# Mictronics/multi-sdr-gps-sim

Hardware: NVIDIA H100
Metric: IQ Msamples/s (higher is better)
Workload: dtype f64 NCO / int32 accumulate / int8 out

## Files before the change

multi-sdr-gps-sim_b200/csrc/synth_lanes.cu:

```cuda
#include <cuda_runtime.h>
#include <stdint.h>

#include "nco_exact.h"
#include "synth_kernels.h"
#include "synth_lanes.h"

namespace gpsb200 {

namespace {

constexpr int kLaneWarps = 16;
constexpr int kLaneChipWords = 36;

struct LaneWin {
    uint32_t s0, s1, s2;
    uint32_t base;
};

struct LaneSteps {
    uint64_t D96, E96;
    uint32_t inv32, e22;
};

template <int CH>
struct LanesSmem {
    static constexpr int kWins = 32 / CH;
    uint32_t chips[CH][kLaneChipWords];
    uint32_t nav[CH][kNavWords];
    alignas(16) LaneWin win[kLaneWarps][kWins][CH];
    alignas(16) uint32_t step[CH];
    LaneSteps steps[CH];
    alignas(16) uint32_t stage[kLaneWarps][kWins * lanes::kWindow];
    uint32_t band[CH][lanes::kBandList + 1];
};
template <int CH>
constexpr size_t lanes_smem_bytes() { return sizeof(LanesSmem<CH>) + (size_t) CH * 2048 + 2048; }

template <int OFF>
__device__ __forceinline__ int table_at(uint32_t p, uint32_t ta) {
    int e;
    asm volatile("{\n\t.reg .b32 i, ad;\n\tshr.b32 i, %1, 23;\n\tmad.lo.u32 ad, i, 4, %2;\n\tld.shared.b32 %0, [ad+%3];\n\t}"
                 : "=r"(e)
                 : "r"(p), "r"(ta), "n"(OFF));
    return e;
}

template <class ChipFn, class NavFn>
__device__ __noinline__ uint3 exact_signs_call(lanes::Anchor an, int w, ChipFn chips, NavFn nav) {
    uint32_t W[3];
    lanes::exact_signs(an, w, chips, nav, W);
    return make_uint3(W[0], W[1], W[2]);
}

__device__ __noinline__ int exact_index_call(lanes::Anchor an, int w, int n) {
    const uint64_t D = lanes::carr_step_fix(an.c);
    const uint64_t P = lanes::carr_fix(an.x0) + (uint64_t) w * ((uint64_t) lanes::kWindow * D);
    return lanes::exact_index(P, D, an, w, n);
}

__device__ __forceinline__ void add_if(int &acc, uint32_t w, uint32_t bit, int e) {
    asm("{\n\t.reg .pred p;\n\t.reg .b32 t;\n\tand.b32 t, %1, %2;\n\tsetp.ne.u32 p, t, 0;\n\t@p add.s32 %0, %0, %3;\n\t}"
        : "+r"(acc)
        : "r"(w), "r"(bit), "r"(e));
}

template <bool IQ16, int CH>
__global__ void __launch_bounds__(kLaneWarps * 32, 2) k_synth_lanes(SynthArgs a) {
    constexpr int WINS = 32 / CH;
    constexpr int SWZ = 32 / CH;
    extern __shared__ __align__(16) unsigned char smem_raw[];
    const uint32_t raw_base = (uint32_t) __cvta_generic_to_shared(smem_raw);
    const uint32_t tab_base = (raw_base + 2047u) & ~2047u;
    int32_t *tab = reinterpret_cast<int32_t *>(smem_raw + (tab_base - raw_base));
    LanesSmem<CH> &sm = *reinterpret_cast<LanesSmem<CH> *>(smem_raw + (tab_base - raw_base) + CH * 2048);
    constexpr uint32_t kFull = 0xFFFFFFFFu;

    const int b = blockIdx.x / a.ctas_per_block;
    const int g = blockIdx.x - b * a.ctas_per_block;
    const int tid = threadIdx.x, nthr = blockDim.x;
    const int lane = tid & 31, warp = tid >> 5;
    const int nchan = a.nchan;
    const BlockChanDev *bc = a.bc + (size_t) b * nchan;

    {
        const int32_t *src = a.atab + (size_t) b * kAtabRows * 32;
        for (int i = tid; i < 512 * CH; i += nthr) {
            const int k = i / CH, c = i - k * CH;
            tab[c * 512 + ((k + c * SWZ) & 511)] = c < nchan ? src[k * 32 + c] : 0;
        }
        for (int i = tid; i < CH * kLaneChipWords; i += nthr) {
            const int c = i / kLaneChipWords, w = i - c * kLaneChipWords;
            uint32_t v = 0;
            if (c < nchan && bc[c].prn > 0) {
                const uint32_t *cw = a.chipbits + bc[c].prn * kChipWords;
                v = w < kChipWords ? cw[w] : __funnelshift_r(cw[w - 32], cw[w - 31], 1);
            }
            sm.chips[c][w] = v;
        }
        for (int i = tid; i < CH * kNavWords; i += nthr) {
            const int c = i / kNavWords, w = i - c * kNavWords;
            uint32_t v = 0;
            if (c < nchan && bc[c].prn > 0) v = a.nav[((size_t) bc[c].frame * a.nav_stride + c) * kNavWords + w];
            sm.nav[c][w] = v;
        }
        if (warp == kLaneWarps - 1 && lane < CH) {
            const bool ok = lane < nchan && bc[lane].prn > 0;
            lanes::ChanRun k;
            lanes::init_steps(k, ok, ok ? bc[lane].c_carr : 0.0, ok ? bc[lane].c_code : 0.0);
            sm.steps[lane] = LaneSteps{k.D96, k.E96, k.inv32, k.e22};
            sm.step[lane] = lanes::fast_step(k);
            lanes::band_residues(lanes::fast_step(k), &sm.band[lane][0]);
        }
    }
    __syncthreads();

    const int ch = lane & (CH - 1), half = lane / CH;
    const bool chan_ok = ch < nchan && bc[ch < nchan ? ch : 0].prn > 0;
    const uint32_t *nav_row = &sm.nav[ch][0];
    const uint32_t *chip_row = &sm.chips[ch][0];
    const uint32_t *band_row = &sm.band[ch][0];
    auto navf = [nav_row](int iw) { return nav_row[iw]; };
    auto chipf = [chip_row](int i) { return chip_row[i]; };
    const uint32_t n0 = (uint32_t) lane, n1 = n0 + 32u, n2 = n0 + 64u;
    const uint32_t sbit = 1u << lanes::sign_pos(lane);
    const int nwin = a.run_samples / lanes::kWindow;
    uint32_t *stage = &sm.stage[warp][0];

    const int run_first = g * a.runs_per_cta;
    const int run_last = min(run_first + a.runs_per_cta, a.nruns);
#pragma unroll 1
    for (int r = run_first + warp; r < run_last; r += kLaneWarps) {
        auto anchor = [&](int c) {
            const RunCkpt k0 = a.ck[((size_t) b * a.nruns + r) * nchan + c];
            return lanes::Anchor{k0.x, k0.y, bc[c].c_carr, bc[c].c_code, k0.nav};
        };
        lanes::ChanRun s;
        auto load_steps = [&]() {
            const LaneSteps k = sm.steps[ch];
            s.D96 = k.D96;
            s.E96 = k.E96;
            s.inv32 = k.inv32;
            s.e22 = k.e22;
        };
        {
            const lanes::Anchor an = chan_ok ? anchor(ch) : lanes::Anchor{0.0, 0.0, 0.0, 0.0, 0u};
            lanes::init_run(s, chan_ok, an.x0, an.y0, an.navpos, an.c, an.d, navf);
        }
        if (WINS == 2 && chan_ok && half == 1) {
            load_steps();
            lanes::advance_window(s, navf);
        }
        const size_t samp0 = (size_t) b * kBlockSamples + (size_t) r * a.run_samples;

#pragma unroll 1
        for (int w = 0; w < nwin; w += WINS) {
            uint32_t flagged;
            {
                uint32_t S[3] = {0u, 0u, 0u};
                uint32_t base = (uint32_t) (ch * SWZ) << 23;
                bool band = false;
                if (chan_ok) load_steps();
                if (chan_ok && w > 0) {
#pragma unroll
                    for (int i = 0; i < WINS; i++) lanes::advance_window(s, navf);
                }
                if (chan_ok && w + half < nwin) {
                    base += lanes::fast_base(s);
                    band = lanes::window_band_risky(band_row, base);
                    if (!lanes::window_signs(s, chipf, navf, S)) {
                        const uint3 e = exact_signs_call(anchor(ch), w + half, chipf, navf);
                        S[0] = e.x;
                        S[1] = e.y;
                        S[2] = e.z;
                    }
                }
                *reinterpret_cast<uint4 *>(&sm.win[warp][half][ch]) = make_uint4(S[0], S[1], S[2], base);
                flagged = __ballot_sync(kFull, band);
            }
            __syncwarp();

#pragma unroll
            for (int hh = 0; hh < WINS; hh++) {
                if (w + hh >= nwin) break;
                const LaneWin *wrow = &sm.win[warp][hh][0];
                int all0 = 0, all1 = 0, all2 = 0, neg0 = 0, neg1 = 0, neg2 = 0;
                const LaneWin *wp = wrow;
                const uint32_t *sp = &sm.step[0];
                uint32_t ta = tab_base;
#pragma unroll 4
                for (int c = 0; c < nchan; c += 2, wp += 2, sp += 2, ta += 2 * 2048u) {
                    const uint4 wa = *reinterpret_cast<const uint4 *>(&wp[0]);
                    const uint4 wb = *reinterpret_cast<const uint4 *>(&wp[1]);
                    const uint2 st = *reinterpret_cast<const uint2 *>(sp);
                    const uint32_t a0 = wa.w + n0 * st.x, a1 = wa.w + n1 * st.x, a2 = wa.w + n2 * st.x;
                    const uint32_t b0 = wb.w + n0 * st.y, b1 = wb.w + n1 * st.y, b2 = wb.w + n2 * st.y;
                    const int ea0 = table_at<0>(a0, ta), eb0 = table_at<2048>(b0, ta);
                    const int ea1 = table_at<0>(a1, ta), eb1 = table_at<2048>(b1, ta);
                    const int ea2 = table_at<0>(a2, ta), eb2 = table_at<2048>(b2, ta);
                    all0 += ea0 + eb0;
                    all1 += ea1 + eb1;
                    all2 += ea2 + eb2;
                    add_if(neg0, wa.x, sbit, ea0);
                    add_if(neg0, wb.x, sbit, eb0);
                    add_if(neg1, wa.y, sbit, ea1);
                    add_if(neg1, wb.y, sbit, eb1);
                    add_if(neg2, wa.z, sbit, ea2);
                    add_if(neg2, wb.z, sbit, eb2);
                }
                int accs[3] = {(int) ((uint32_t) all0 - 2u * (uint32_t) neg0), (int) ((uint32_t) all1 - 2u * (uint32_t) neg1),
                               (int) ((uint32_t) all2 - 2u * (uint32_t) neg2)};
                for (uint32_t m = WINS == 1 ? flagged : (flagged >> (hh * CH)) & 0xFFFFu; m != 0u; m &= m - 1u) {
                    const int c = __ffs((int) m) - 1;
                    const uint4 wv = *reinterpret_cast<const uint4 *>(&wrow[c]);
                    const uint32_t st = sm.step[c];
                    const uint32_t p0 = wv.w + n0 * st, p1 = wv.w + n1 * st, p2 = wv.w + n2 * st;
                    const bool risky = lanes::fast_risky(p0) | lanes::fast_risky(p1) | lanes::fast_risky(p2);
                    if (!risky) continue;
                    const lanes::Anchor ac = anchor(c);
                    const uint32_t ps[3] = {p0, p1, p2}, sw[3] = {wv.x, wv.y, wv.z};
#pragma unroll
                    for (int j = 0; j < 3; j++) {
                        if (!lanes::fast_risky(ps[j])) continue;
                        const int kf = (int) (ps[j] >> 23);
                        const int k = exact_index_call(ac, w + hh, 32 * j + lane);
                        const int fix = tab[c * 512 + ((k + c * SWZ) & 511)] - tab[c * 512 + kf];
                        accs[j] += (sw[j] & sbit) ? -fix : fix;
                    }
                }
#pragma unroll
                for (int j = 0; j < 3; j++) {
                    const int p = accs[j];
                    const int iv = (int) (short) (p & 0xFFFF);
                    const int qv = (p - iv) >> 16;
                    const int n = hh * lanes::kWindow + 32 * j + lane;
                    if (IQ16) {
                        stage[n] = ((uint32_t) iv & 0xFFFFu) | ((uint32_t) qv << 16);
                    } else {
                        reinterpret_cast<uint16_t *>(stage)[n] =
                            (uint16_t) ((((uint32_t) (iv >> 4)) & 0xFFu) | ((((uint32_t) (qv >> 4)) & 0xFFu) << 8));
                    }
                }
            }
            __syncwarp();
            {
                const int nsamp = (nwin - w >= WINS ? WINS : 1) * lanes::kWindow;
                const int nvec = nsamp * (IQ16 ? 4 : 2) / 16;
                uint4 *dst = reinterpret_cast<uint4 *>(reinterpret_cast<char *>(a.out) +
                                                       (samp0 + (size_t) w * lanes::kWindow) * (IQ16 ? 4 : 2));
                const uint4 *srcv = reinterpret_cast<const uint4 *>(stage);
                for (int i = lane; i < nvec; i += 32) dst[i] = srcv[i];
            }
        }
    }
}

}

bool synth_lanes_applicable(const SynthArgs &a) {
    return a.lanes && a.nchan <= 32 && a.run_samples % lanes::kWindow == 0 && a.run_samples <= lanes::kMaxRun;
}

static int device_sms() {
    int dev = 0, n = 0;
    if (cudaGetDevice(&dev) != cudaSuccess || cudaDeviceGetAttribute(&n, cudaDevAttrMultiProcessorCount, dev) != cudaSuccess)
        return 132;
    return n;
}

static void lanes_shape(const SynthArgs &a, int *ctas_per_block, int *runs_per_cta) {
    int per_block = (40 * 2 * device_sms() + a.nblk - 1) / a.nblk;
    if (per_block > 16) per_block = 16;
    if (per_block < 1) per_block = 1;
    int per_cta = (a.nruns + per_block - 1) / per_block;
    per_cta = (per_cta + kLaneWarps - 1) / kLaneWarps * kLaneWarps;
    per_block = (a.nruns + per_cta - 1) / per_cta;
    *ctas_per_block = per_block;
    *runs_per_cta = per_cta;
}

template <bool IQ16, int CH>
static cudaError_t launch_lanes_t(const SynthArgs &a, cudaStream_t s) {
    const size_t smem = lanes_smem_bytes<CH>();
    cudaError_t e = cudaFuncSetAttribute(k_synth_lanes<IQ16, CH>, cudaFuncAttributeMaxDynamicSharedMemorySize, (int) smem);
    if (e != cudaSuccess) return e;
    k_synth_lanes<IQ16, CH><<<a.nblk * a.ctas_per_block, kLaneWarps * 32, smem, s>>>(a);
    return cudaGetLastError();
}

cudaError_t launch_synth_lanes(const SynthArgs &a_in, cudaStream_t s) {
    SynthArgs a = a_in;
    lanes_shape(a, &a.ctas_per_block, &a.runs_per_cta);
    if (a.nchan <= 16) return a.iq16 ? launch_lanes_t<true, 16>(a, s) : launch_lanes_t<false, 16>(a, s);
    return a.iq16 ? launch_lanes_t<true, 32>(a, s) : launch_lanes_t<false, 32>(a, s);
}

void synth_lanes_launch_shape(const SynthArgs &a, int *ctas, int *threads, size_t *smem, int *ctas_per_block,
                              int *runs_per_cta) {
    int per_block, per_cta;
    lanes_shape(a, &per_block, &per_cta);
    *ctas = a.nblk * per_block;
    *threads = kLaneWarps * 32;
    *smem = a.nchan <= 16 ? lanes_smem_bytes<16>() : lanes_smem_bytes<32>();
    *ctas_per_block = per_block;
    *runs_per_cta = per_cta;
}

}
```

multi-sdr-gps-sim_b200/csrc/synth_lanes.h:

```cpp
#pragma once
#include <stdint.h>

#include "nco_exact.h"

namespace gpsb200 {
namespace lanes {

constexpr int kWindow = 96;
constexpr int kMaxRun = 2400;
constexpr uint64_t kOne54 = 1ull << 54;
constexpr uint64_t kCodeWrap54 = 1023ull << 54;
constexpr uint64_t kBandCode = 1ull << 22;
constexpr uint64_t kBandCarr = 1ull << 23;
constexpr uint32_t kBandFast = 128;

GPSB_HD bool code_step_ok(double c_code) { return c_code >= 0.33855 && c_code < 0.34340; }

GPSB_HD uint64_t carr_fix(double x) { return (x >= 0.0 && x < 1.0) ? (uint64_t) (x * 0x1p64) : 0; }
GPSB_HD uint64_t carr_step_fix(double c) {
    const double a = c < 0.0 ? -c : c;
    const uint64_t m = (uint64_t) (a * 0x1p64);
    return c < 0.0 ? (uint64_t) 0 - m : m;
}
GPSB_HD uint64_t code_fix(double y) { return (uint64_t) (y * 0x1p54); }

GPSB_HD uint32_t funnel_r(uint32_t lo, uint32_t hi, int sh) {
#if defined(__CUDA_ARCH__)
    return __funnelshift_r(lo, hi, sh);
#else
    return sh ? (lo >> sh) | (hi << (32 - sh)) : lo;
#endif
}

struct ChanRun {
    uint64_t P, D;
    uint64_t Y, E;
    uint64_t D96, E96;
    uint32_t inv32;
    uint32_t e22;
    int iword, ibit, icode, dbit;
    bool active;
};

struct Anchor {
    double x0, y0, c, d;
    uint32_t navpos;
};

template <class NavFn>
GPSB_HD int nav_bit_at(NavFn nav, int iw, int ib) {
    const uint32_t w = nav(iw < 60 ? iw : 59);
    return (int) ((w >> (29 - ib)) & 1u);
}

GPSB_HD void init_steps(ChanRun &s, bool active, double c, double d) {
    s.D = carr_step_fix(c);
    s.E = code_fix(d);
    s.D96 = (uint64_t) kWindow * s.D;
    s.E96 = (uint64_t) kWindow * s.E;
    const uint64_t d3 = 3 * s.E - kOne54;
    s.inv32 = active ? (uint32_t) (0x1p79 / (double) d3) : 0u;
    s.e22 = (uint32_t) (s.E >> 22);
}

template <class NavFn>
GPSB_HD void init_run(ChanRun &s, bool active, double x, double y, uint32_t navpos, double c, double d, NavFn nav) {
    s.active = active;
    s.iword = (int) (navpos & 0xFF);
    s.ibit = (int) ((navpos >> 8) & 0xFF);
    s.icode = (int) ((navpos >> 16) & 0xFF);
    s.P = carr_fix(x);
    s.Y = code_fix(y);
    init_steps(s, active, c, d);
    s.dbit = active ? nav_bit_at(nav, s.iword, s.ibit) : 0;
}

GPSB_HD uint32_t mulhi32(uint32_t a, uint32_t b) {
#if defined(__CUDA_ARCH__)
    return __umulhi(a, b);
#else
    return (uint32_t) (((uint64_t) a * b) >> 32);
#endif
}

GPSB_HD bool window_signs_fp64(const ChanRun &s, uint32_t c_lo, uint32_t c_hi, int j0, uint32_t S[3]) {
    const uint64_t d3 = (s.E96 >> 5) - kOne54;
    const double rinv = 1.0 / (double) d3;
    const double tband = (double) kBandCode * rinv + 0x1p-40;
    bool certain = true;
#pragma unroll
    for (int r = 0; r < 3; r++) {
        const uint64_t phi = s.Y + (uint64_t) r * s.E;
        const int J = (int) (phi >> 54) - j0;
        const uint64_t F = phi & (kOne54 - 1);
        const double t = (double) (kOne54 - F) * rinv;
        const double tf = t < 64.0 ? (double) (int) t : 64.0;
        const int qs = (int) tf + 1;
        certain &= F >= kBandCode;
        if (qs <= 32) certain &= (t - tf >= tband) & (tf + 1.0 - t >= tband);
        const uint32_t lowm = qs >= 32 ? 0xFFFFFFFFu : ((1u << qs) - 1u);
        const uint32_t a = funnel_r(c_lo, c_hi, J), b = funnel_r(c_lo, c_hi, J + 1);
        S[r] = (a & lowm) | (b & ~lowm);
    }
    return certain;
}

GPSB_HD int sign_pos(int i) { return 11 * (i % 3) + i / 3; }

GPSB_HD void sample_words(const uint32_t S[3], uint32_t W[3]) {
    W[0] = (S[0] & 0x7FFu) | ((S[1] & 0x7FFu) << 11) | (S[2] << 22);
    W[1] = ((S[2] >> 10) & 0x7FFu) | (((S[0] >> 11) & 0x7FFu) << 11) | ((S[1] >> 11) << 22);
    W[2] = (S[1] >> 21) | ((S[2] >> 21) << 11) | ((S[0] >> 22) << 22);
}

template <class ChipFn, class NavFn>
GPSB_HD bool window_signs(const ChanRun &s, ChipFn chips, NavFn nav, uint32_t W[3], bool force_fp64 = false) {
    const int j0 = (int) (s.Y >> 54);
    const int wi = j0 >> 5, sh = j0 & 31;
    const uint32_t w0 = chips(wi), w1 = chips(wi + 1), w2 = chips(wi + 2);
    uint32_t c_lo = funnel_r(w0, w1, sh), c_hi = funnel_r(w1, w2, sh);
    if (s.dbit) {
        c_lo = ~c_lo;
        c_hi = ~c_hi;
    }
    const int pw = 1023 - j0;
    if (pw < 64 && s.icode == 19) {
        int ib = s.ibit + 1, iw = s.iword;
        if (ib >= 30) {
            ib = 0;
            ++iw;
        }
        if (nav_bit_at(nav, iw, ib) != s.dbit) {
            if (pw < 32) {
                c_lo ^= 0xFFFFFFFFu << pw;
                c_hi = ~c_hi;
            } else {
                c_hi ^= 0xFFFFFFFFu << (pw - 32);
            }
        }
    }
    const uint32_t f0 = (uint32_t) (s.Y >> 22);
    const uint32_t sh1 = funnel_r(c_lo, c_hi, 1), sh2 = funnel_r(c_lo, c_hi, 2);
    bool certain = !force_fp64;
    uint32_t S[3];
#pragma unroll
    for (int r = 0; r < 3; r++) {
        const uint32_t fr = f0 + (uint32_t) r * s.e22;
        const bool J = fr < f0;
        certain &= fr + 4u >= 8u;
        const uint32_t t25 = mulhi32(~fr - 2u, s.inv32);
        const uint32_t fl = t25 >> 25, frac = t25 & ((1u << 25) - 1u);
        certain &= (fl >= 32u) | ((frac >= 16u) & (frac < (1u << 25) - 16u));
        const uint32_t lowm = fl >= 31u ? 0xFFFFFFFFu : ((2u << fl) - 1u);
        const uint32_t a = J ? sh1 : c_lo, b = J ? sh2 : sh1;
        S[r] = (a & lowm) | (b & ~lowm);
    }
    if (!certain && !window_signs_fp64(s, c_lo, c_hi, j0, S)) return false;
    sample_words(S, W);
    return true;
}

template <class NavFn>
GPSB_HD void advance_window(ChanRun &s, NavFn nav) {
    s.P += s.D96;
    const uint64_t y_old = s.Y;
    s.Y += s.E96;
    if (s.Y < y_old || s.Y >= kCodeWrap54) {
        s.Y -= kCodeWrap54;
        if (++s.icode >= 20) {
            s.icode = 0;
            if (++s.ibit >= 30) {
                s.ibit = 0;
                ++s.iword;
            }
            s.dbit = nav_bit_at(nav, s.iword, s.ibit);
        }
    }
}

template <class ChipFn, class NavFn>
GPSB_HD void exact_signs(const Anchor &an, int w, ChipFn chips, NavFn nav, uint32_t W[3]) {
    double y = an.y0;
    int iword = (int) (an.navpos & 0xFF), ibit = (int) ((an.navpos >> 8) & 0xFF), icode = (int) ((an.navpos >> 16) & 0xFF);
    int64_t periods = 0;
    nco_advance<NCO_CODE>(y, an.d, (int64_t) w * kWindow, periods);
    nav_advance(iword, ibit, icode, periods);
    int dbit = nav_bit_at(nav, iword, ibit);
    W[0] = W[1] = W[2] = 0;
    for (int n = 0; n < kWindow; n++) {
        const int j = (int) y;
        const uint32_t chip = (chips(j >> 5) >> (j & 31)) & 1u;
        const uint32_t flag = chip ^ (uint32_t) dbit;
        W[n >> 5] |= flag << sign_pos(n & 31);
        int64_t p = 0;
        nco_step<NCO_CODE>(y, an.d, p);
        if (p) {
            if (++icode >= 20) {
                icode = 0;
                if (++ibit >= 30) {
                    ibit = 0;
                    ++iword;
                }
                dbit = nav_bit_at(nav, iword, ibit);
            }
        }
    }
}

GPSB_HD int exact_index(uint64_t P, uint64_t D, const Anchor &an, int w, int n, bool force_walk = false) {
    const uint64_t m = P + (uint64_t) n * D;
    const uint64_t frac = m & ((1ull << 55) - 1);
    if (!force_walk && frac >= kBandCarr && frac <= (1ull << 55) - kBandCarr) return (int) (m >> 55);
    double x = an.x0;
    int64_t dummy = 0;
    nco_advance<NCO_CARRIER>(x, an.c, (int64_t) w * kWindow + n, dummy);
#if defined(__CUDA_ARCH__)
    return __double2loint(__dadd_rz(x, 8796093022208.0)) & 511;
#else
    return (int) (x * 512.0) & 511;
#endif
}

GPSB_HD uint32_t fast_base(const ChanRun &s) { return (uint32_t) (s.P >> 32) - 1u; }
GPSB_HD uint32_t fast_step(const ChanRun &s) { return (uint32_t) (s.D >> 32); }
GPSB_HD bool fast_risky(uint32_t p) { return (((~p) << 9) < (kBandFast << 9)); }

constexpr uint32_t kMod23 = 1u << 23;
constexpr int kBandList = 128;
constexpr uint32_t kBandPad = kMod23;

GPSB_HD int band_distinct(uint32_t u) {
    if (u == 0) return 1;
    const uint32_t period = kMod23 / (u & (0u - u));
    return period < (uint32_t) kWindow ? (int) period : kWindow;
}

GPSB_HD void band_residues(uint32_t step, uint32_t *R) {
    const uint32_t u = step & (kMod23 - 1);
    const int m = band_distinct(u);
    int a = 0, b = 0;
    uint32_t ra = kMod23, rb = 0;
    for (int n = 1; n < m; n++) {
        const uint32_t r = ((uint32_t) n * u) & (kMod23 - 1);
        if (r < ra) ra = r, a = n;
        if (r > rb) rb = r, b = n;
    }
    const uint32_t db = kMod23 - rb;
    int n = 0;
    uint32_t r = 0;
    for (int k = 0; k < m; k++) {
        R[k] = r;
        if (n + a < m) {
            n += a;
            r += ra;
        } else if (n >= b) {
            n -= b;
            r += db;
        } else {
            n += a - b;
            r += ra + db;
        }
    }
    for (int k = m; k < kBandList; k++) R[k] = kBandPad;
}

GPSB_HD bool window_band_risky(const uint32_t *R, uint32_t base) {
    const uint32_t t = (0u - kBandFast - base) & (kMod23 - 1);
    const uint32_t te = t + kBandFast;
    uint32_t i = 0, lo = 0;
#pragma unroll
    for (uint32_t s = kBandList / 2; s > 0; s >>= 1) {
        const uint32_t v = R[i + s - 1];
        if (v < te) {
            i += s;
            lo = v;
        }
    }
    return lo >= t;
}

}
}
```

Baseline: 69210.

## Pack nav state, specialize channel loop, drop table alignment, simplify IQ packing

Packs the per-channel nav position (word, bit, code, data bit) into one 32-bit register to reduce register pressure. It adds a compile-time-unrolled channel-sum path for the full 32-channel case. It also removes the 2 KB shared-memory alignment padding for the amplitude table, simplifies the I/Q unpack and int8 packing arithmetic, and hoists the output pointer so the store loop uses a fixed trip count. Dropping the alignment changes the table addresses and may alter shared-memory bank behaviour. The packed nav field needs extra shift and mask work on window advance.

```diff
diff --git a/multi-sdr-gps-sim_b200/csrc/synth_lanes.cu b/multi-sdr-gps-sim_b200/csrc/synth_lanes.cu
--- a/multi-sdr-gps-sim_b200/csrc/synth_lanes.cu
+++ b/multi-sdr-gps-sim_b200/csrc/synth_lanes.cu
@@ -10,6 +10,7 @@
 namespace {
 
 constexpr int kLaneWarps = 16;
+constexpr int kLaneCtas = 2;
 constexpr int kLaneChipWords = 36;
 
 struct LaneWin {
@@ -34,7 +35,7 @@
     uint32_t band[CH][lanes::kBandList + 1];
 };
 template <int CH>
-constexpr size_t lanes_smem_bytes() { return sizeof(LanesSmem<CH>) + (size_t) CH * 2048 + 2048; }
+constexpr size_t lanes_smem_bytes() { return sizeof(LanesSmem<CH>) + (size_t) CH * 2048; }
 
 template <int OFF>
 __device__ __forceinline__ int table_at(uint32_t p, uint32_t ta) {
@@ -64,15 +65,46 @@
         : "r"(w), "r"(bit), "r"(e));
 }
 
+template <int NC>
+__device__ __forceinline__ void window_sums(const LaneWin *wp, const uint32_t *sp, uint32_t ta, int nchan, uint32_t n0,
+                                            uint32_t sbit, int accs[3]) {
+    const int nc = NC > 0 ? NC : nchan;
+    const uint32_t n1 = n0 + 32u, n2 = n0 + 64u;
+    int all0 = 0, all1 = 0, all2 = 0, neg0 = 0, neg1 = 0, neg2 = 0;
+#pragma unroll 4
+    for (int c = 0; c < nc; c += 2, wp += 2, sp += 2, ta += 2 * 2048u) {
+        const uint4 wa = *reinterpret_cast<const uint4 *>(&wp[0]);
+        const uint4 wb = *reinterpret_cast<const uint4 *>(&wp[1]);
+        const uint2 st = *reinterpret_cast<const uint2 *>(sp);
+        const uint32_t a0 = wa.w + n0 * st.x, a1 = wa.w + n1 * st.x, a2 = wa.w + n2 * st.x;
+        const uint32_t b0 = wb.w + n0 * st.y, b1 = wb.w + n1 * st.y, b2 = wb.w + n2 * st.y;
+        const int ea0 = table_at<0>(a0, ta), eb0 = table_at<2048>(b0, ta);
+        const int ea1 = table_at<0>(a1, ta), eb1 = table_at<2048>(b1, ta);
+        const int ea2 = table_at<0>(a2, ta), eb2 = table_at<2048>(b2, ta);
+        all0 += ea0 + eb0;
+        all1 += ea1 + eb1;
+        all2 += ea2 + eb2;
+        add_if(neg0, wa.x, sbit, ea0);
+        add_if(neg0, wb.x, sbit, eb0);
+        add_if(neg1, wa.y, sbit, ea1);
+        add_if(neg1, wb.y, sbit, eb1);
+        add_if(neg2, wa.z, sbit, ea2);
+        add_if(neg2, wb.z, sbit, eb2);
+    }
+    accs[0] = (int) ((uint32_t) all0 - 2u * (uint32_t) neg0);
+    accs[1] = (int) ((uint32_t) all1 - 2u * (uint32_t) neg1);
+    accs[2] = (int) ((uint32_t) all2 - 2u * (uint32_t) neg2);
+}
+
 template <bool IQ16, int CH>
-__global__ void __launch_bounds__(kLaneWarps * 32, 2) k_synth_lanes(SynthArgs a) {
+__global__ void __launch_bounds__(kLaneWarps * 32, kLaneCtas) k_synth_lanes(SynthArgs a) {
     constexpr int WINS = 32 / CH;
     constexpr int SWZ = 32 / CH;
+    constexpr int BYTES = IQ16 ? 4 : 2;
     extern __shared__ __align__(16) unsigned char smem_raw[];
-    const uint32_t raw_base = (uint32_t) __cvta_generic_to_shared(smem_raw);
-    const uint32_t tab_base = (raw_base + 2047u) & ~2047u;
-    int32_t *tab = reinterpret_cast<int32_t *>(smem_raw + (tab_base - raw_base));
-    LanesSmem<CH> &sm = *reinterpret_cast<LanesSmem<CH> *>(smem_raw + (tab_base - raw_base) + CH * 2048);
+    int32_t *tab = reinterpret_cast<int32_t *>(smem_raw);
+    LanesSmem<CH> &sm = *reinterpret_cast<LanesSmem<CH> *>(smem_raw + CH * 2048);
+    const uint32_t tab_base = (uint32_t) __cvta_generic_to_shared(smem_raw);
     constexpr uint32_t kFull = 0xFFFFFFFFu;
 
     const int b = blockIdx.x / a.ctas_per_block;
@@ -150,7 +182,8 @@
             load_steps();
             lanes::advance_window(s, navf);
         }
-        const size_t samp0 = (size_t) b * kBlockSamples + (size_t) r * a.run_samples;
+        uint4 *dst = reinterpret_cast<uint4 *>(reinterpret_cast<char *>(a.out) +
+                                               ((size_t) b * kBlockSamples + (size_t) r * a.run_samples) * BYTES);
 
 #pragma unroll 1
         for (int w = 0; w < nwin; w += WINS) {
@@ -183,32 +216,11 @@
             for (int hh = 0; hh < WINS; hh++) {
                 if (w + hh >= nwin) break;
                 const LaneWin *wrow = &sm.win[warp][hh][0];
-                int all0 = 0, all1 = 0, all2 = 0, neg0 = 0, neg1 = 0, neg2 = 0;
-                const LaneWin *wp = wrow;
-                const uint32_t *sp = &sm.step[0];
-                uint32_t ta = tab_base;
-#pragma unroll 4
-                for (int c = 0; c < nchan; c += 2, wp += 2, sp += 2, ta += 2 * 2048u) {
-                    const uint4 wa = *reinterpret_cast<const uint4 *>(&wp[0]);
-                    const uint4 wb = *reinterpret_cast<const uint4 *>(&wp[1]);
-                    const uint2 st = *reinterpret_cast<const uint2 *>(sp);
-                    const uint32_t a0 = wa.w + n0 * st.x, a1 = wa.w + n1 * st.x, a2 = wa.w + n2 * st.x;
-                    const uint32_t b0 = wb.w + n0 * st.y, b1 = wb.w + n1 * st.y, b2 = wb.w + n2 * st.y;
-                    const int ea0 = table_at<0>(a0, ta), eb0 = table_at<2048>(b0, ta);
-                    const int ea1 = table_at<0>(a1, ta), eb1 = table_at<2048>(b1, ta);
-                    const int ea2 = table_at<0>(a2, ta), eb2 = table_at<2048>(b2, ta);
-                    all0 += ea0 + eb0;
-                    all1 += ea1 + eb1;
-                    all2 += ea2 + eb2;
-                    add_if(neg0, wa.x, sbit, ea0);
-                    add_if(neg0, wb.x, sbit, eb0);
-                    add_if(neg1, wa.y, sbit, ea1);
-                    add_if(neg1, wb.y, sbit, eb1);
-                    add_if(neg2, wa.z, sbit, ea2);
-                    add_if(neg2, wb.z, sbit, eb2);
-                }
-                int accs[3] = {(int) ((uint32_t) all0 - 2u * (uint32_t) neg0), (int) ((uint32_t) all1 - 2u * (uint32_t) neg1),
-                               (int) ((uint32_t) all2 - 2u * (uint32_t) neg2)};
+                int accs[3];
+                if (CH == 32 && nchan == CH)
+                    window_sums<CH>(wrow, &sm.step[0], tab_base, nchan, n0, sbit, accs);
+                else
+                    window_sums<0>(wrow, &sm.step[0], tab_base, nchan, n0, sbit, accs);
                 for (uint32_t m = WINS == 1 ? flagged : (flagged >> (hh * CH)) & 0xFFFFu; m != 0u; m &= m - 1u) {
                     const int c = __ffs((int) m) - 1;
                     const uint4 wv = *reinterpret_cast<const uint4 *>(&wrow[c]);
@@ -229,26 +241,24 @@
                 }
 #pragma unroll
                 for (int j = 0; j < 3; j++) {
-                    const int p = accs[j];
-                    const int iv = (int) (short) (p & 0xFFFF);
-                    const int qv = (p - iv) >> 16;
+                    const uint32_t p = (uint32_t) accs[j];
+                    const uint32_t x = p + ((p & 0x8000u) << 1);
                     const int n = hh * lanes::kWindow + 32 * j + lane;
-                    if (IQ16) {
-                        stage[n] = ((uint32_t) iv & 0xFFFFu) | ((uint32_t) qv << 16);
-                    } else {
-                        reinterpret_cast<uint16_t *>(stage)[n] =
-                            (uint16_t) ((((uint32_t) (iv >> 4)) & 0xFFu) | ((((uint32_t) (qv >> 4)) & 0xFFu) << 8));
-                    }
+                    if (IQ16)
+                        stage[n] = x;
+                    else
+                        reinterpret_cast<uint16_t *>(stage)[n] = (uint16_t) (((p >> 4) & 0xFFu) | ((x >> 12) & 0xFF00u));
                 }
             }
             __syncwarp();
             {
-                const int nsamp = (nwin - w >= WINS ? WINS : 1) * lanes::kWindow;
-                const int nvec = nsamp * (IQ16 ? 4 : 2) / 16;
-                uint4 *dst = reinterpret_cast<uint4 *>(reinterpret_cast<char *>(a.out) +
-                                                       (samp0 + (size_t) w * lanes::kWindow) * (IQ16 ? 4 : 2));
+                constexpr int kVec = WINS * lanes::kWindow * BYTES / 16;
+                const int nvec = WINS == 1 || nwin - w >= WINS ? kVec : kVec / WINS;
                 const uint4 *srcv = reinterpret_cast<const uint4 *>(stage);
-                for (int i = lane; i < nvec; i += 32) dst[i] = srcv[i];
+#pragma unroll
+                for (int i = lane; i < ((kVec + 31) & ~31); i += 32)
+                    if (i < nvec) dst[i] = srcv[i];
+                dst += kVec;
             }
         }
     }
@@ -268,7 +278,7 @@
 }
 
 static void lanes_shape(const SynthArgs &a, int *ctas_per_block, int *runs_per_cta) {
-    int per_block = (40 * 2 * device_sms() + a.nblk - 1) / a.nblk;
+    int per_block = (40 * kLaneCtas * device_sms() + a.nblk - 1) / a.nblk;
     if (per_block > 16) per_block = 16;
     if (per_block < 1) per_block = 1;
     int per_cta = (a.nruns + per_block - 1) / per_block;
diff --git a/multi-sdr-gps-sim_b200/csrc/synth_lanes.h b/multi-sdr-gps-sim_b200/csrc/synth_lanes.h
--- a/multi-sdr-gps-sim_b200/csrc/synth_lanes.h
+++ b/multi-sdr-gps-sim_b200/csrc/synth_lanes.h
@@ -38,9 +38,14 @@
     uint64_t D96, E96;
     uint32_t inv32;
     uint32_t e22;
-    int iword, ibit, icode, dbit;
+    uint32_t nav;
     bool active;
 };
+
+GPSB_HD int nav_iword(uint32_t nav) { return (int) (nav & 0xFF); }
+GPSB_HD int nav_ibit(uint32_t nav) { return (int) ((nav >> 8) & 0xFF); }
+GPSB_HD int nav_icode(uint32_t nav) { return (int) ((nav >> 16) & 0xFF); }
+GPSB_HD uint32_t nav_dbit(uint32_t nav) { return nav >> 24; }
 
 struct Anchor {
     double x0, y0, c, d;
@@ -66,13 +71,11 @@
 template <class NavFn>
 GPSB_HD void init_run(ChanRun &s, bool active, double x, double y, uint32_t navpos, double c, double d, NavFn nav) {
     s.active = active;
-    s.iword = (int) (navpos & 0xFF);
-    s.ibit = (int) ((navpos >> 8) & 0xFF);
-    s.icode = (int) ((navpos >> 16) & 0xFF);
+    s.nav = navpos & 0xFFFFFFu;
     s.P = carr_fix(x);
     s.Y = code_fix(y);
     init_steps(s, active, c, d);
-    s.dbit = active ? nav_bit_at(nav, s.iword, s.ibit) : 0;
+    if (active) s.nav |= (uint32_t) nav_bit_at(nav, nav_iword(s.nav), nav_ibit(s.nav)) << 24;
 }
 
 GPSB_HD uint32_t mulhi32(uint32_t a, uint32_t b) {
@@ -119,18 +122,19 @@
     const int wi = j0 >> 5, sh = j0 & 31;
     const uint32_t w0 = chips(wi), w1 = chips(wi + 1), w2 = chips(wi + 2);
     uint32_t c_lo = funnel_r(w0, w1, sh), c_hi = funnel_r(w1, w2, sh);
-    if (s.dbit) {
+    const int dbit = (int) nav_dbit(s.nav);
+    if (dbit) {
         c_lo = ~c_lo;
         c_hi = ~c_hi;
     }
     const int pw = 1023 - j0;
-    if (pw < 64 && s.icode == 19) {
-        int ib = s.ibit + 1, iw = s.iword;
+    if (pw < 64 && nav_icode(s.nav) == 19) {
+        int ib = nav_ibit(s.nav) + 1, iw = nav_iword(s.nav);
         if (ib >= 30) {
             ib = 0;
             ++iw;
         }
-        if (nav_bit_at(nav, iw, ib) != s.dbit) {
+        if (nav_bit_at(nav, iw, ib) != dbit) {
             if (pw < 32) {
                 c_lo ^= 0xFFFFFFFFu << pw;
                 c_hi = ~c_hi;
@@ -167,14 +171,17 @@
     s.Y += s.E96;
     if (s.Y < y_old || s.Y >= kCodeWrap54) {
         s.Y -= kCodeWrap54;
-        if (++s.icode >= 20) {
-            s.icode = 0;
-            if (++s.ibit >= 30) {
-                s.ibit = 0;
-                ++s.iword;
+        int icode = nav_icode(s.nav) + 1, ibit = nav_ibit(s.nav), iword = nav_iword(s.nav);
+        uint32_t dbit = nav_dbit(s.nav);
+        if (icode >= 20) {
+            icode = 0;
+            if (++ibit >= 30) {
+                ibit = 0;
+                ++iword;
             }
-            s.dbit = nav_bit_at(nav, s.iword, s.ibit);
-        }
+            dbit = (uint32_t) nav_bit_at(nav, iword, ibit);
+        }
+        s.nav = (uint32_t) iword | ((uint32_t) ibit << 8) | ((uint32_t) icode << 16) | (dbit << 24);
     }
 }
 
```

Measured after the change: 71300 (median of 6 runs). +3.0%, better.
